# nytdevansh/Optimized-Sparse-Retrieval-for-High-Performance-RAG-Pipelines

Hardware: AMD Instinct MI355X
Metric: queries/sec + achieved HBM GB/s, batch BM25 top-k=100 (higher is better)
Workload: dtype f32

## Files before the change

include/sparse_rx.h:

```cpp
#ifndef SPARSE_RX_H
#define SPARSE_RX_H

#include <stdint.h>

#ifdef __cplusplus
extern "C" {
#endif

#define SRX_VERSION 301

typedef enum {
    SRX_OK = 0,
    SRX_ERR_INVALID = -1,
    SRX_ERR_HIP = -2,
    SRX_ERR_NOMEM = -3,
    SRX_ERR_NODEVICE = -4
} srx_status;

typedef enum {
    SRX_VAL_F32 = 0,
    SRX_VAL_F16 = 1
} srx_val_type;

#define SRX_MAX_K 1024
#define SRX_MAX_TILE_LOG2 14
#define SRX_BLOCK_PAD 256

typedef struct {
    int32_t device;
    int32_t val_type;
    int64_t n_docs;
    int64_t vocab;
    int64_t nnz;
    int64_t n_blocks;
    int64_t doc_base;
    int32_t tile_log2;
    int32_t n_tiles;
    int32_t unit_tiles;
    int32_t reserved0;
    const int64_t *term_ptr;
    const int32_t *post;
    const int32_t *tile_skip;
    const float *idf;
    const float *term_bound;
    const int32_t *post16;
} srx_index_desc;

typedef struct srx_index srx_index;

typedef enum {
    SRX_DBG_TIER2_ONLY = 8,
    SRX_DBG_NO_TERM_BOUND = 16,
    SRX_DBG_NO_FLAT_TILES = 128,
    SRX_DBG_BLOCK_MERGE = 256,
    SRX_DBG_NO_WAVE_DENSE = 2048,
    SRX_DBG_WAVE_DENSE_MASKED = 4096,
    SRX_DBG_WAVE_DENSE_GENERAL = 8192,
    SRX_DBG_ALL = SRX_DBG_TIER2_ONLY | SRX_DBG_NO_TERM_BOUND | SRX_DBG_NO_FLAT_TILES | SRX_DBG_BLOCK_MERGE | SRX_DBG_NO_WAVE_DENSE |
                  SRX_DBG_WAVE_DENSE_MASKED | SRX_DBG_WAVE_DENSE_GENERAL
} srx_debug_bits;

typedef struct {
    int32_t supertile_log2;
    int32_t target_blocks;
    int32_t profile;
    int32_t reserved;
    int32_t unit_tiles;
} srx_search_opts;

int srx_version(void);
const char *srx_last_error(void);
int srx_limits(int32_t *h_out4);
int srx_device_count(void);

int srx_index_create(const srx_index_desc *h_desc, srx_index **h_out);
void srx_index_destroy(srx_index *ix);
int srx_index_set_opts(srx_index *ix, const srx_search_opts *h_opts);

int64_t srx_search_workspace_bytes(const srx_index *ix, int32_t nq, int32_t k);

int srx_search(srx_index *ix, const int32_t *q_ptr, const int32_t *q_term, const float *q_weight, int32_t nq,
               int32_t k, int32_t *out_doc, float *out_score, int32_t *out_count, void *workspace,
               int64_t workspace_bytes, void *stream);

int64_t srx_merge_workspace_bytes(int32_t nq, int32_t n_lists, int32_t k);
int srx_merge_topk(int32_t device, const int32_t *in_doc, const float *in_score, const int32_t *in_count,
                   int32_t nq, int32_t n_lists, int32_t k, int32_t gathered, int32_t *out_doc, float *out_score,
                   int32_t *out_count, void *workspace, int64_t workspace_bytes, void *stream);

int srx_merge_topk_packed(int32_t device, const int32_t *packed, int32_t nq, int32_t n_lists, int32_t k,
                          int32_t *out_doc, float *out_score, int32_t *out_count, void *workspace,
                          int64_t workspace_bytes, void *stream);

int srx_search_packed(srx_index *ix, const int32_t *q_ptr, const int32_t *q_term, const float *q_weight, int32_t nq,
                      int32_t k, int32_t *out_packed, void *workspace, int64_t workspace_bytes, void *stream);
int srx_merge_topk_packed_out(int32_t device, const int32_t *packed, int32_t nq, int32_t n_lists, int32_t k,
                              int32_t *out_packed, void *workspace, int64_t workspace_bytes, void *stream);

int srx_search_after(srx_index *ix, const int32_t *q_ptr, const int32_t *q_term, const float *q_weight, int32_t nq,
                     int32_t k, const int32_t *after_doc, const float *after_score, int32_t *out_doc, float *out_score,
                     int32_t *out_count, void *workspace, int64_t workspace_bytes, void *stream);
int srx_search_after_packed(srx_index *ix, const int32_t *q_ptr, const int32_t *q_term, const float *q_weight, int32_t nq,
                            int32_t k, const int32_t *after_doc, const float *after_score, int32_t *out_packed,
                            void *workspace, int64_t workspace_bytes, void *stream);


int srx_build_impacts(int32_t device, const float *tf, const int32_t *post_doc, const float *doc_len, int64_t nnz,
                      double k1, double b, double avgdl, float *out_impact, void *stream);

int srx_build_tile_skip(int32_t device, const int64_t *term_ptr, const int32_t *post_doc, int64_t vocab,
                        int32_t n_tiles, int32_t tile_log2, int32_t *out_skip, void *stream);

int32_t srx_auto_unit_tiles(int64_t n_docs, int64_t vocab, int64_t nnz, int32_t tile_log2);

int srx_build_blocks(int32_t device, int32_t val_type, const int64_t *term_ptr, const int32_t *post_term,
                     const int32_t *post_doc, const void *post_val, const int32_t *skip, const int64_t *runpad,
                     int64_t vocab, int64_t nnz, int32_t n_tiles, int32_t tile_log2, int32_t unit_tiles, int32_t *out_post,
                     int32_t *out_skip, int64_t *out_term_ptr, int64_t n_blocks, void *stream);

int srx_build_sum_duplicates(int32_t device, const int64_t *first, int64_t n_groups, const float *val, float *out_sum, void *stream);

int srx_build_term_bounds(int32_t device, int32_t val_type, const int64_t *term_ptr, const void *post_val, int64_t vocab,
                          const int32_t *ks, int32_t nk, float *out_bound, int32_t *neg_flag, void *stream);

int srx_build_compact(int32_t device, int32_t val_type, const int32_t *post, int64_t n_blocks_total, int32_t tile_log2,
                      int32_t unit_tiles, int32_t *out_post16, void *stream);

int srx_memcpy_async(void *dst, const void *src, int64_t bytes, void *stream);

int64_t srx_dense_workspace_bytes(int32_t nq, int64_t n_docs, int32_t k);
int srx_dense_search_i8(int32_t device, const int8_t *corpus, const float *corpus_scale, int64_t n_docs, int32_t dim,
                        const int8_t *queries, const float *query_scale, int32_t nq, int32_t k, int64_t doc_base,
                        int32_t *out_doc, float *out_score, int32_t *out_count, void *workspace, int64_t workspace_bytes,
                        void *stream);
int64_t srx_dense_packed_bytes(int64_t n_rows, int32_t dim);
int srx_dense_pack_i8(int32_t device, const int8_t *rows, int64_t n_rows, int32_t dim, void *out_packed, void *stream);
int srx_dense_search_i8_packed(int32_t device, const void *corpus_packed, const float *corpus_scale, int64_t n_docs, int32_t dim,
                               const int8_t *queries, const float *query_scale, int32_t nq, int32_t k, int64_t doc_base,
                               int32_t *out_doc, float *out_score, int32_t *out_count, void *workspace,
                               int64_t workspace_bytes, void *stream);

int64_t srx_dense_f32_workspace_bytes(int32_t nq, int64_t n_docs, int32_t k);
int srx_dense_search_f32(int32_t device, const float *emb, int64_t n_docs, int32_t dim, const float *queries, int32_t nq,
                         int32_t k, int64_t doc_base, int32_t *out_doc, float *out_score, int32_t *out_count,
                         void *workspace, int64_t workspace_bytes, void *stream, float score_offset);

int srx_dense_search_u8(int32_t device, const uint8_t *corpus, const float *corpus_scales, int64_t n_docs, int32_t dim,
                        const float *queries, int32_t nq, int32_t k, int64_t doc_base, int32_t *out_doc, float *out_score,
                        int32_t *out_count, void *workspace, int64_t workspace_bytes, void *stream);

typedef enum {
    SRX_FUSE_WEIGHTED = 0,
    SRX_FUSE_RRF = 1
} srx_fuse_mode;
int srx_fuse_topk(int32_t device, const int32_t *a_doc, const float *a_score, const int32_t *a_count, int32_t ka,
                  const int32_t *b_doc, const float *b_score, const int32_t *b_count, int32_t kb, int32_t nq, int32_t k,
                  int32_t mode, float weight_a, float weight_b, float rrf_c, int32_t *out_doc, float *out_score,
                  int32_t *out_count, void *stream);

int srx_score_docs(const srx_index_desc *h_desc, const int32_t *q_ptr, const int32_t *q_term, const float *q_weight, int32_t nq,
                   const int32_t *cand_doc, const int32_t *cand_count, int32_t m, float *out_score, void *stream);

int srx_profile_read(srx_index *ix, float *h_ms4);

#ifdef __cplusplus
}
#endif
#endif
```

optimized-sparse-retrieval-for-high-performance-rag-pipelines_amd/_capi.py:

```python
from __future__ import annotations

import ctypes
import os
import shutil
import subprocess
from typing import Optional

_PKG_DIR = os.path.dirname(os.path.abspath(__file__))
_ROOT = os.path.dirname(_PKG_DIR)
LIB_PATH = os.path.join(_PKG_DIR, "libsparse_rx.so")
CSRC_DIR = os.path.join(_PKG_DIR, "csrc")
SOURCES = ["wave_kernel.hip", "tier2_kernel.hip", "merge.hip", "build.hip", "sparse_rx.hip", "dense.hip", "fuse.hip",
           "score_docs.hip"]
SRC_PATH = os.path.join(CSRC_DIR, "wave_kernel.hip")
INCLUDE_DIR = os.path.join(_ROOT, "include")

HIPCC_FLAGS = ["--offload-arch=gfx950", "-O3", "-ffp-contract=off", "-fPIC", "-fvisibility=hidden", "-std=c++17"]

SRX_VAL_F32, SRX_VAL_F16 = 0, 1
SRX_FUSE_WEIGHTED, SRX_FUSE_RRF = 0, 1
SRX_MAX_K = 1024


class SparseRxUnavailable(RuntimeError):
    """libsparse_rx.so is not built / not loadable (the HIP engine is mandatory)."""


class SparseRxError(RuntimeError):
    """A C-ABI call returned a negative status."""


class IndexDesc(ctypes.Structure):
    _fields_ = [("device", ctypes.c_int32), ("val_type", ctypes.c_int32), ("n_docs", ctypes.c_int64),
                ("vocab", ctypes.c_int64), ("nnz", ctypes.c_int64), ("n_blocks", ctypes.c_int64), ("doc_base", ctypes.c_int64),
                ("tile_log2", ctypes.c_int32), ("n_tiles", ctypes.c_int32), ("unit_tiles", ctypes.c_int32),
                ("reserved0", ctypes.c_int32), ("term_ptr", ctypes.c_void_p), ("post", ctypes.c_void_p),
                ("tile_skip", ctypes.c_void_p), ("idf", ctypes.c_void_p), ("term_bound", ctypes.c_void_p),
                ("post16", ctypes.c_void_p)]


class SearchOpts(ctypes.Structure):
    _fields_ = [("supertile_log2", ctypes.c_int32), ("target_blocks", ctypes.c_int32), ("profile", ctypes.c_int32),
                ("reserved", ctypes.c_int32), ("unit_tiles", ctypes.c_int32)]


_VP, _I32, _I64, _DBL = ctypes.c_void_p, ctypes.c_int32, ctypes.c_int64, ctypes.c_double
SYMBOLS = {
    "srx_version": (ctypes.c_int, []),
    "srx_last_error": (ctypes.c_char_p, []),
    "srx_limits": (ctypes.c_int, [ctypes.POINTER(_I32)]),
    "srx_device_count": (ctypes.c_int, []),
    "srx_index_create": (ctypes.c_int, [ctypes.POINTER(IndexDesc), ctypes.POINTER(_VP)]),
    "srx_index_destroy": (None, [_VP]),
    "srx_index_set_opts": (ctypes.c_int, [_VP, ctypes.POINTER(SearchOpts)]),
    "srx_search_workspace_bytes": (_I64, [_VP, _I32, _I32]),
    "srx_search": (ctypes.c_int, [_VP, _VP, _VP, _VP, _I32, _I32, _VP, _VP, _VP, _VP, _I64, _VP]),
    "srx_search_after": (ctypes.c_int, [_VP, _VP, _VP, _VP, _I32, _I32, _VP, _VP, _VP, _VP, _VP, _VP, _I64, _VP]),
    "srx_search_after_packed": (ctypes.c_int, [_VP, _VP, _VP, _VP, _I32, _I32, _VP, _VP, _VP, _VP, _I64, _VP]),
    "srx_merge_workspace_bytes": (_I64, [_I32, _I32, _I32]),
    "srx_merge_topk": (ctypes.c_int, [_I32, _VP, _VP, _VP, _I32, _I32, _I32, _I32, _VP, _VP, _VP, _VP, _I64, _VP]),
    "srx_merge_topk_packed": (ctypes.c_int, [_I32, _VP, _I32, _I32, _I32, _VP, _VP, _VP, _VP, _I64, _VP]),
    "srx_search_packed": (ctypes.c_int, [_VP, _VP, _VP, _VP, _I32, _I32, _VP, _VP, _I64, _VP]),
    "srx_merge_topk_packed_out": (ctypes.c_int, [_I32, _VP, _I32, _I32, _I32, _VP, _VP, _I64, _VP]),
    "srx_dense_workspace_bytes": (_I64, [_I32, _I64, _I32]),
    "srx_dense_search_i8": (ctypes.c_int, [_I32, _VP, _VP, _I64, _I32, _VP, _VP, _I32, _I32, _I64, _VP, _VP, _VP, _VP, _I64, _VP]),
    "srx_dense_packed_bytes": (_I64, [_I64, _I32]),
    "srx_dense_pack_i8": (ctypes.c_int, [_I32, _VP, _I64, _I32, _VP, _VP]),
    "srx_dense_search_i8_packed": (ctypes.c_int, [_I32, _VP, _VP, _I64, _I32, _VP, _VP, _I32, _I32, _I64, _VP, _VP, _VP, _VP, _I64, _VP]),
    "srx_dense_f32_workspace_bytes": (_I64, [_I32, _I64, _I32]),
    "srx_dense_search_f32": (ctypes.c_int, [_I32, _VP, _I64, _I32, _VP, _I32, _I32, _I64, _VP, _VP, _VP, _VP, _I64, _VP, ctypes.c_float]),
    "srx_dense_search_u8": (ctypes.c_int, [_I32, _VP, _VP, _I64, _I32, _VP, _I32, _I32, _I64, _VP, _VP, _VP, _VP, _I64, _VP]),
    "srx_fuse_topk": (ctypes.c_int, [_I32, _VP, _VP, _VP, _I32, _VP, _VP, _VP, _I32, _I32, _I32, _I32, ctypes.c_float, ctypes.c_float,
                                     ctypes.c_float, _VP, _VP, _VP, _VP]),
    "srx_score_docs": (ctypes.c_int, [ctypes.POINTER(IndexDesc), _VP, _VP, _VP, _I32, _VP, _VP, _I32, _VP, _VP]),
    "srx_build_impacts": (ctypes.c_int, [_I32, _VP, _VP, _VP, _I64, _DBL, _DBL, _DBL, _VP, _VP]),
    "srx_build_tile_skip": (ctypes.c_int, [_I32, _VP, _VP, _I64, _I32, _I32, _VP, _VP]),
    "srx_memcpy_async": (ctypes.c_int, [_VP, _VP, _I64, _VP]),
    "srx_auto_unit_tiles": (_I32, [_I64, _I64, _I64, _I32]),
    "srx_build_blocks": (ctypes.c_int, [_I32, _I32, _VP, _VP, _VP, _VP, _VP, _VP, _I64, _I64, _I32, _I32, _I32, _VP, _VP, _VP, _I64, _VP]),
    "srx_build_compact": (ctypes.c_int, [_I32, _I32, _VP, _I64, _I32, _I32, _VP, _VP]),
    "srx_build_term_bounds": (ctypes.c_int, [_I32, _I32, _VP, _VP, _I64, _VP, _I32, _VP, _VP, _VP]),
    "srx_build_sum_duplicates": (ctypes.c_int, [_I32, _VP, _I64, _VP, _VP, _VP]),
    "srx_profile_read": (ctypes.c_int, [_VP, ctypes.POINTER(ctypes.c_float)]),
}

_lib: Optional[ctypes.CDLL] = None


def kernel_sources_sha256() -> str:
    import hashlib
    h = hashlib.sha256()
    for f in ["wave_kernel.hip", "tier2_kernel.hip", "merge.hip", "srx_common.h"]:
        with open(os.path.join(CSRC_DIR, f), "rb") as fh:
            h.update(fh.read())
    return h.hexdigest()


def _deps():
    return [os.path.join(CSRC_DIR, f) for f in SOURCES] + [os.path.join(CSRC_DIR, "srx_common.h"),
                                                            os.path.join(INCLUDE_DIR, "sparse_rx.h")]


def build_library(force: bool = False, verbose: bool = False) -> str:
    if not force and os.path.exists(LIB_PATH) and os.path.getmtime(LIB_PATH) >= max(os.path.getmtime(p) for p in _deps()):
        return LIB_PATH
    hipcc = shutil.which("hipcc") or "/opt/rocm/bin/hipcc"
    if not os.path.exists(hipcc):
        raise SparseRxUnavailable("hipcc not found: cannot build libsparse_rx.so")
    objdir = os.path.join(CSRC_DIR, "build")
    os.makedirs(objdir, exist_ok=True)
    newest_hdr = max(os.path.getmtime(os.path.join(CSRC_DIR, "srx_common.h")), os.path.getmtime(os.path.join(INCLUDE_DIR, "sparse_rx.h")))
    procs, objs = [], []
    for f in SOURCES:
        src, obj = os.path.join(CSRC_DIR, f), os.path.join(objdir, f.replace(".hip", ".o"))
        objs.append(obj)
        if not force and os.path.exists(obj) and os.path.getmtime(obj) >= max(os.path.getmtime(src), newest_hdr):
            continue
        cmd = [hipcc, *HIPCC_FLAGS, f"-I{INCLUDE_DIR}", f"-I{CSRC_DIR}", "-c", "-o", obj, src]
        if verbose:
            print(" ".join(cmd))
        procs.append((f, subprocess.Popen(cmd)))
    for f, p in procs:
        if p.wait() != 0:
            raise subprocess.CalledProcessError(p.returncode, f"hipcc -c {f}")
    cmd = [hipcc, "--offload-arch=gfx950", "-shared", "-fPIC", "-fvisibility=hidden", "-o", LIB_PATH, *objs]
    if verbose:
        print(" ".join(cmd))
    subprocess.run(cmd, check=True)
    return LIB_PATH


def lib() -> ctypes.CDLL:
    global _lib
    if _lib is not None:
        return _lib
    if not os.path.exists(LIB_PATH):
        raise SparseRxUnavailable(
            f"{LIB_PATH} is missing: build it with `python -c 'import __graft_entry__ as g; g.build()'` "
            "(hipcc --offload-arch=gfx950).  There is no CPU fallback.")
    try:
        L = ctypes.CDLL(LIB_PATH)
    except OSError as e:
        raise SparseRxUnavailable(f"cannot load {LIB_PATH}: {e}") from e
    for name, (res, args) in SYMBOLS.items():
        try:
            f = getattr(L, name)
        except AttributeError as e:
            raise SparseRxUnavailable(f"{LIB_PATH} does not export {name}") from e
        f.restype = res
        f.argtypes = args
    _lib = L
    return L


def check(rc: int, what: str) -> int:
    if rc < 0:
        msg = lib().srx_last_error()
        text = msg.decode("utf-8", "replace") if msg else ""
        if rc == -1:
            raise ValueError(f"{what}: {text}")
        raise SparseRxError(f"{what} failed ({rc}): {text}")
    return rc


def limits():
    out = (ctypes.c_int32 * 4)()
    check(lib().srx_limits(out), "srx_limits")
    return {"max_k": out[0], "max_tile_log2": out[1], "hash_cap": out[2], "threads": out[3]}
```

optimized-sparse-retrieval-for-high-performance-rag-pipelines_amd/csrc/sparse_rx.hip:

```cpp

#include "srx_common.h"

thread_local char srx_g_err[512] = "";

#define SRX_TRY(expr)                  \
    do {                               \
        const int rc_ = (expr);        \
        if (rc_ != SRX_OK) return rc_; \
    } while (0)

namespace {
constexpr int PROF_SLOTS = 256;
constexpr int PROF_EVENTS = 4;
struct SearchProfile {
    hipEvent_t *ev;
    hipEvent_t *cur;
    int n;
    int64_t calls;
    int64_t searches;

    int begin(int every) {
        cur = nullptr;
        if (every <= 0 || (searches++ % every) != 0) return SRX_OK;
        if (!ev) {
            ev = new (std::nothrow) hipEvent_t[PROF_EVENTS * PROF_SLOTS];
            if (!ev) return fail(SRX_ERR_NOMEM, "srx_search: host allocation failed%s");
            for (int i = 0; i < PROF_EVENTS * PROF_SLOTS; ++i) HIP_TRY(hipEventCreate(&ev[i]));
        }
        cur = ev + PROF_EVENTS * (int)(calls % PROF_SLOTS);
        return SRX_OK;
    }
    int mark(int i, hipStream_t stream) {
        if (cur) HIP_TRY(hipEventRecord(cur[i], stream));
        return SRX_OK;
    }
    void end() {
        if (!cur) return;
        ++calls;
        if (n < PROF_SLOTS) ++n;
    }
    int read(float *h_ms4) {
        if (n == 0 || !ev) return fail(SRX_ERR_INVALID, "srx_profile_read: no profiled srx_search has run%s");
        static constexpr int FROM[4] = {0, 1, 2, 0}, TO[4] = {1, 2, 3, 3};
        double acc[4] = {0, 0, 0, 0};
        for (int i = 0; i < n; ++i) {
            const hipEvent_t *e = ev + PROF_EVENTS * (int)((calls - 1 - i) % PROF_SLOTS);
            HIP_TRY(hipEventSynchronize(e[3]));
            for (int j = 0; j < 4; ++j) {
                float ms = 0;
                HIP_TRY(hipEventElapsedTime(&ms, e[FROM[j]], e[TO[j]]));
                acc[j] += ms;
            }
        }
        for (int j = 0; j < 4; ++j) h_ms4[j] = (float)(acc[j] / n);
        const int averaged = n;
        n = 0;
        return averaged;
    }
    void destroy() {
        if (!ev) return;
        for (int i = 0; i < PROF_EVENTS * PROF_SLOTS; ++i) (void)hipEventDestroy(ev[i]);
        delete[] ev;
    }
};
}

struct srx_index {
    srx_index_desc d;
    srx_search_opts opts;
    SearchProfile prof;
    int *h_hint;
    int *d_hint;
};

SRX_API int srx_version(void) { return SRX_VERSION; }
SRX_API const char *srx_last_error(void) { return g_err; }

SRX_API int srx_limits(int32_t *h_out4) {
    if (!h_out4) return fail(SRX_ERR_INVALID, "srx_limits: null output%s");
    h_out4[0] = KMAX;
    h_out4[1] = SRX_MAX_TILE_LOG2;
    h_out4[2] = HASH_CAP;
    h_out4[3] = THREADS;
    return SRX_OK;
}

SRX_API int srx_device_count(void) {
    int n = 0;
    hipError_t e = hipGetDeviceCount(&n);
    if (e != hipSuccess) return fail(SRX_ERR_NODEVICE, "hipGetDeviceCount: %s", hipGetErrorString(e));
    return n;
}

SRX_API int srx_index_create(const srx_index_desc *d, srx_index **out) {
    if (!d || !out) return fail(SRX_ERR_INVALID, "srx_index_create: null argument%s");
    if (d->n_docs <= 0 || d->n_docs >= 0x7FFFFFFFll) return fail(SRX_ERR_INVALID, "srx_index_create: n_docs out of range%s");
    if (d->doc_base < 0 || d->doc_base + d->n_docs >= 0x7FFFFFFFll)
        return fail(SRX_ERR_INVALID, "srx_index_create: doc_base + n_docs must fit int32%s");
    if (d->vocab <= 0 || d->nnz < 0) return fail(SRX_ERR_INVALID, "srx_index_create: bad vocab / nnz%s");
    if (d->tile_log2 < 6 || d->tile_log2 > SRX_MAX_TILE_LOG2)
        return fail(SRX_ERR_INVALID, "srx_index_create: tile_log2 must be in [6, 14]%s");
    const int64_t nt = (d->n_docs + (1ll << d->tile_log2) - 1) >> d->tile_log2;
    if (d->n_tiles != nt) return fail(SRX_ERR_INVALID, "srx_index_create: n_tiles != ceil(n_docs / 2^tile_log2)%s");
    if (d->val_type != SRX_VAL_F32 && d->val_type != SRX_VAL_F16) return fail(SRX_ERR_INVALID, "srx_index_create: bad val_type%s");
    if (d->unit_tiles < 1 || d->unit_tiles > MAX_TPS) return fail(SRX_ERR_INVALID, "srx_index_create: unit_tiles must be in [1, 64]%s");
    if (d->n_blocks < 0 || d->n_blocks * 4 < d->nnz) return fail(SRX_ERR_INVALID, "srx_index_create: n_blocks does not cover nnz%s");
    if (!d->term_ptr || !d->tile_skip || !d->idf || (!d->post && !d->post16))
        return fail(SRX_ERR_INVALID, "srx_index_create: null index array%s");
    if (!d->post && ((int64_t)d->unit_tiles << d->tile_log2) > W_UNIT_MAX_DOCS)
        return fail(SRX_ERR_INVALID, "srx_index_create: an index without canonical blocks needs units of <= 49152 docs (the compact copy)%s");
    int ndev = 0;
    HIP_TRY(hipGetDeviceCount(&ndev));
    if (d->device < 0 || d->device >= ndev) return fail(SRX_ERR_NODEVICE, "srx_index_create: device ordinal not visible%s");
    srx_index *ix = new (std::nothrow) srx_index();
    if (!ix) return fail(SRX_ERR_NOMEM, "srx_index_create: host allocation failed%s");
    ix->d = *d;
    int *h = nullptr, *dev = nullptr;
    const bool pinned = hipSetDevice(d->device) == hipSuccess && hipHostMalloc((void **)&h, 64, hipHostMallocMapped) == hipSuccess;
    if (pinned && hipHostGetDevicePointer((void **)&dev, h, 0) == hipSuccess) {
        h[0] = -1;
        ix->h_hint = h;
        ix->d_hint = dev;
    } else {
        if (pinned) (void)hipHostFree(h);
        (void)hipGetLastError();
    }
    *out = ix;
    return SRX_OK;
}

SRX_API void srx_index_destroy(srx_index *ix) {
    if (!ix) return;
    ix->prof.destroy();
    if (ix->h_hint) (void)hipHostFree(ix->h_hint);
    delete ix;
}

SRX_API int srx_index_set_opts(srx_index *ix, const srx_search_opts *o) {
    if (!ix || !o) return fail(SRX_ERR_INVALID, "srx_index_set_opts: null argument%s");
    if (o->supertile_log2 != 0 && (o->supertile_log2 < ix->d.tile_log2 || o->supertile_log2 > ix->d.tile_log2 + 6))
        return fail(SRX_ERR_INVALID, "srx_index_set_opts: supertile_log2 must be in [tile_log2, tile_log2+6]%s");
    if (o->unit_tiles < 0 || o->unit_tiles > MAX_TPS) return fail(SRX_ERR_INVALID, "srx_index_set_opts: unit_tiles must be in [0, 64]%s");
    if (o->target_blocks < 0) return fail(SRX_ERR_INVALID, "srx_index_set_opts: target_blocks < 0%s");
    if (o->reserved & ~SRX_DBG_ALL)
        return fail(SRX_ERR_INVALID, "srx_index_set_opts: reserved takes only the bits 8, 16, 128, 256, 2048, 4096, 8192%s");
    ix->opts = *o;
    return SRX_OK;
}

namespace {
struct Plan {
    int tpu, n_super, n_splits, n_whole, ovf_words, lists_per_q;
};

Plan make_plan(const srx_index *ix, int nq, int k) {
    Plan p;
    const srx_index_desc &d = ix->d;
    int tpu;
    if (ix->opts.unit_tiles > 0) {
        tpu = ix->opts.unit_tiles;
    } else if (ix->opts.supertile_log2 != 0) {
        tpu = 1 << (ix->opts.supertile_log2 - d.tile_log2);
    } else {
        tpu = d.unit_tiles;
    }
    if (tpu < 1) tpu = 1;
    if (tpu > MAX_TPS) tpu = MAX_TPS;
    p.tpu = tpu;
    p.n_super = (int)((d.n_tiles + tpu - 1) / tpu);
    const int target = ix->opts.target_blocks > 0 ? ix->opts.target_blocks : 3072;
    int ns = target / (nq > 0 ? nq : 1);
    int n_whole = 0;
    if (nq > target) {
        n_whole = nq / target * target;
        const int tail = nq - n_whole;
        ns = tail > 0 ? target / tail : 1;
        if (ns > 4) ns = 4;
        if (ns < 2) ns = 2;
        if (tail == 0) ns = 1;
    }
    if (ns < 1) ns = 1;
    if (ns > p.n_super) ns = p.n_super;
    const int cap = (MERGE_NPT * THREADS) / (2 * (k > 0 ? k : 1));
    if (ns > cap) ns = cap;
    if (ns < 1) ns = 1;
    if (ns == 1) n_whole = 0;
    p.n_splits = ns;
    p.n_whole = n_whole;
    p.ovf_words = (p.n_super + 31) / 32;
    p.lists_per_q = 2 * ns;
    return p;
}
}

namespace {
struct SearchWs {
    int32_t *cand_doc;
    float *cand_score;
    int32_t *cand_count;
    unsigned *ovf;
    unsigned *done;
    int *work;
    int64_t lists, items;
    int64_t bytes;
};
SearchWs search_ws(void *base, const Plan &p, int nq, int k) {
    SearchWs w;
    w.lists = (int64_t)nq * p.lists_per_q;
    w.items = (int64_t)p.n_whole + (int64_t)(nq - p.n_whole) * p.n_splits;
    w.cand_doc = (int32_t *)base;
    w.cand_score = (float *)(w.cand_doc + w.lists * k);
    w.cand_count = (int32_t *)(w.cand_score + w.lists * k);
    w.ovf = (unsigned *)(w.cand_count + w.lists);
    w.done = w.ovf + w.items * p.ovf_words;
    w.work = (int *)(w.done + (nq - p.n_whole));
    w.bytes = (int64_t)((char *)(w.work + 1 + w.items) - (char *)base) + 256;
    return w;
}
}

SRX_API int64_t srx_search_workspace_bytes(const srx_index *ix, int32_t nq, int32_t k) {
    if (!ix || nq < 0 || k <= 0 || k > KMAX) return fail(SRX_ERR_INVALID, "srx_search_workspace_bytes: bad argument%s");
    return search_ws(nullptr, make_plan(ix, nq, k), nq, k).bytes;
}

namespace {
IndexView index_view(const srx_index *ix, bool after) {
    const srx_index_desc &d = ix->d;
    IndexView v;
    v.term_ptr = d.term_ptr; v.post = d.post; v.post16 = d.post16; v.tile_skip = d.tile_skip; v.idf = d.idf;
    v.term_bound = ((ix->opts.reserved & SRX_DBG_NO_TERM_BOUND) || after) ? nullptr : d.term_bound;
    v.n_docs = d.n_docs; v.vocab = d.vocab; v.zero_block = d.n_blocks;
    v.tile_log2 = d.tile_log2; v.n_tiles = d.n_tiles; v.unit_tiles = d.unit_tiles;
    return v;
}

int search_impl(srx_index *ix, const int32_t *q_ptr, const int32_t *q_term, const float *q_weight, int32_t nq,
                int32_t k, const srx_rows &out, void *workspace, int64_t workspace_bytes, void *stream_v,
                const int32_t *after_doc = nullptr, const float *after_score = nullptr) {
    if (!ix) return fail(SRX_ERR_INVALID, "srx_search: null index%s");
    if ((after_doc == nullptr) != (after_score == nullptr)) return fail(SRX_ERR_INVALID, "srx_search_after: after_doc and after_score go together%s");
    if (nq < 0 || k <= 0 || k > KMAX) return fail(SRX_ERR_INVALID, "srx_search: need nq >= 0 and 1 <= k <= 1024%s");
    if (nq == 0) return SRX_OK;
    if (!q_ptr || !out.doc || !out.score || !out.count) return fail(SRX_ERR_INVALID, "srx_search: null query / output pointer%s");
    const Plan p = make_plan(ix, nq, k);
    const SearchWs w = search_ws(workspace, p, nq, k);
    if (!workspace || workspace_bytes < w.bytes) return fail(SRX_ERR_NOMEM, "srx_search: workspace too small%s");
    hipStream_t stream = (hipStream_t)stream_v;
    HIP_TRY(hipSetDevice(ix->d.device));
    if (ix->d.post == nullptr && p.tpu != ix->d.unit_tiles)
        return fail(SRX_ERR_INVALID, "srx_search: this index keeps no canonical blocks: a unit other than the one it was built for cannot be served%s");
    if (w.lists > 0x7FFFFFFFll) return fail(SRX_ERR_INVALID, "srx_search: nq * splits overflows the grid%s");

    const bool tier2_only = (ix->opts.reserved & SRX_DBG_TIER2_ONLY) != 0 || after_score != nullptr || p.tpu != ix->d.unit_tiles;
    srx_score_launch sl;
    srx_wave_launch &a = sl.w;
    a.ix = index_view(ix, after_score != nullptr);
    a.q_ptr = q_ptr; a.q_term = q_term; a.q_weight = q_weight;
    a.nq = nq; a.k = k; a.n_splits = p.n_splits; a.n_whole = p.n_whole; a.n_super = p.n_super;
    a.dbg = ix->opts.reserved | (tier2_only ? SRX_DBG_TIER2_ONLY : 0);
    a.ovf = w.ovf; a.ovf_words = p.ovf_words; a.lists_per_q = p.lists_per_q; a.work = w.work; a.done = w.done;
    a.cand_doc = w.cand_doc; a.cand_score = w.cand_score; a.cand_count = w.cand_count;
    a.doc_base = ix->d.doc_base; a.out_doc = out.doc; a.out_score = out.score; a.out_count = out.count;
    a.out_row_stride = out.row_stride; a.out_cnt_stride = out.cnt_stride;
    sl.tpu = p.tpu; sl.after_doc = after_doc; sl.after_score = after_score; sl.hint = ix->d_hint;

    SRX_TRY(ix->prof.begin(ix->opts.profile));
    HIP_TRY(hipMemsetAsync(w.done, 0, (size_t)(1 + (nq - p.n_whole)) * 4, stream));
    SRX_TRY(ix->prof.mark(0, stream));
    SRX_TRY(srx_launch_wave_kernel(sl.w, ix->d.val_type, w.items, stream));
    SRX_TRY(ix->prof.mark(1, stream));
    const int hint = ix->h_hint ? *(volatile int *)ix->h_hint : -1;
    const int64_t t2_full = w.items < 1024 ? w.items : 1024;
    const bool t2_small = hint == 0 && t2_full > 128 && !tier1_serves_nothing(a.ix, k, p.tpu, a.dbg);
    SRX_TRY(srx_launch_score_kernel(sl, ix->d.val_type, (unsigned)(t2_small ? 128 : t2_full), stream));
    SRX_TRY(ix->prof.mark(2, stream));
    if (nq > p.n_whole)
        SRX_TRY(srx_launch_final_merge(srx_plain_rows(w.cand_doc, w.cand_score, w.cand_count, k), nq, p.lists_per_q, k, 0, ix->d.doc_base,
                                       out, nullptr, p.n_whole, 1, (a.dbg & SRX_DBG_BLOCK_MERGE) != 0, stream));
    SRX_TRY(ix->prof.mark(3, stream));
    ix->prof.end();
    return SRX_OK;
}
}

SRX_API int srx_search(srx_index *ix, const int32_t *q_ptr, const int32_t *q_term, const float *q_weight, int32_t nq,
                       int32_t k, int32_t *out_doc, float *out_score, int32_t *out_count, void *workspace,
                       int64_t workspace_bytes, void *stream_v) {
    return search_impl(ix, q_ptr, q_term, q_weight, nq, k, srx_plain_rows(out_doc, out_score, out_count, k), workspace,
                       workspace_bytes, stream_v);
}

SRX_API int srx_search_packed(srx_index *ix, const int32_t *q_ptr, const int32_t *q_term, const float *q_weight,
                              int32_t nq, int32_t k, int32_t *out_packed, void *workspace, int64_t workspace_bytes,
                              void *stream_v) {
    if (!out_packed || k <= 0) return fail(SRX_ERR_INVALID, "srx_search_packed: bad argument%s");
    return search_impl(ix, q_ptr, q_term, q_weight, nq, k, srx_packed_rows<float>(out_packed, k), workspace, workspace_bytes, stream_v);
}

SRX_API int srx_search_after(srx_index *ix, const int32_t *q_ptr, const int32_t *q_term, const float *q_weight, int32_t nq,
                             int32_t k, const int32_t *after_doc, const float *after_score, int32_t *out_doc, float *out_score,
                             int32_t *out_count, void *workspace, int64_t workspace_bytes, void *stream_v) {
    if (!after_doc || !after_score) return fail(SRX_ERR_INVALID, "srx_search_after: null bound arrays%s");
    return search_impl(ix, q_ptr, q_term, q_weight, nq, k, srx_plain_rows(out_doc, out_score, out_count, k), workspace,
                       workspace_bytes, stream_v, after_doc, after_score);
}

SRX_API int srx_search_after_packed(srx_index *ix, const int32_t *q_ptr, const int32_t *q_term, const float *q_weight,
                                    int32_t nq, int32_t k, const int32_t *after_doc, const float *after_score,
                                    int32_t *out_packed, void *workspace, int64_t workspace_bytes, void *stream_v) {
    if (!out_packed || k <= 0 || !after_doc || !after_score) return fail(SRX_ERR_INVALID, "srx_search_after_packed: bad argument%s");
    return search_impl(ix, q_ptr, q_term, q_weight, nq, k, srx_packed_rows<float>(out_packed, k), workspace, workspace_bytes, stream_v,
                       after_doc, after_score);
}

SRX_API int srx_profile_read(srx_index *ix, float *h_ms4) {
    if (!ix || !h_ms4) return fail(SRX_ERR_INVALID, "srx_profile_read: null argument%s");
    return ix->prof.read(h_ms4);
}

SRX_API int srx_memcpy_async(void *dst, const void *src, int64_t bytes, void *stream_v) {
    if (bytes < 0 || (bytes > 0 && (!dst || !src))) return fail(SRX_ERR_INVALID, "srx_memcpy_async: bad argument%s");
    if (bytes == 0) return SRX_OK;
    HIP_TRY(hipMemcpyAsync(dst, src, (size_t)bytes, hipMemcpyDefault, (hipStream_t)stream_v));
    return SRX_OK;
}
```

Before: 9.319 million.

## Add new tier-1 wave kernel with prefetch pipeline and bitmap duplicate detection

Adds a separate tier-1 scoring kernel, launched by default in place of the previous wave kernel, which stays reachable through a new debug bit. The new kernel reads query-term metadata with a scalar prologue and prefetches tile-skip bounds and posting blocks two supertiles ahead. Duplicate docs are found with an LDS bitmap plus atomicOr, and dense units are sent to tier 2. The aim is to hide load latency and lower per-unit overhead, at the price of a large new code path with its own register and LDS pressure.

```diff
diff --git a/include/sparse_rx.h b/include/sparse_rx.h
--- a/include/sparse_rx.h
+++ b/include/sparse_rx.h
@@ -56,8 +56,9 @@
     SRX_DBG_NO_WAVE_DENSE = 2048,
     SRX_DBG_WAVE_DENSE_MASKED = 4096,
     SRX_DBG_WAVE_DENSE_GENERAL = 8192,
+    SRX_DBG_TIER1_PREVIOUS = 16384,
     SRX_DBG_ALL = SRX_DBG_TIER2_ONLY | SRX_DBG_NO_TERM_BOUND | SRX_DBG_NO_FLAT_TILES | SRX_DBG_BLOCK_MERGE | SRX_DBG_NO_WAVE_DENSE |
-                  SRX_DBG_WAVE_DENSE_MASKED | SRX_DBG_WAVE_DENSE_GENERAL
+                  SRX_DBG_WAVE_DENSE_MASKED | SRX_DBG_WAVE_DENSE_GENERAL | SRX_DBG_TIER1_PREVIOUS
 } srx_debug_bits;
 
 typedef struct {
diff --git a/optimized-sparse-retrieval-for-high-performance-rag-pipelines_amd/_capi.py b/optimized-sparse-retrieval-for-high-performance-rag-pipelines_amd/_capi.py
--- a/optimized-sparse-retrieval-for-high-performance-rag-pipelines_amd/_capi.py
+++ b/optimized-sparse-retrieval-for-high-performance-rag-pipelines_amd/_capi.py
@@ -10,7 +10,7 @@
 _ROOT = os.path.dirname(_PKG_DIR)
 LIB_PATH = os.path.join(_PKG_DIR, "libsparse_rx.so")
 CSRC_DIR = os.path.join(_PKG_DIR, "csrc")
-SOURCES = ["wave_kernel.hip", "tier2_kernel.hip", "merge.hip", "build.hip", "sparse_rx.hip", "dense.hip", "fuse.hip",
+SOURCES = ["tier1_kernel.hip", "wave_kernel.hip", "tier2_kernel.hip", "merge.hip", "build.hip", "sparse_rx.hip", "dense.hip", "fuse.hip",
            "score_docs.hip"]
 SRC_PATH = os.path.join(CSRC_DIR, "wave_kernel.hip")
 INCLUDE_DIR = os.path.join(_ROOT, "include")
diff --git a/optimized-sparse-retrieval-for-high-performance-rag-pipelines_amd/csrc/sparse_rx.hip b/optimized-sparse-retrieval-for-high-performance-rag-pipelines_amd/csrc/sparse_rx.hip
--- a/optimized-sparse-retrieval-for-high-performance-rag-pipelines_amd/csrc/sparse_rx.hip
+++ b/optimized-sparse-retrieval-for-high-performance-rag-pipelines_amd/csrc/sparse_rx.hip
@@ -1,5 +1,7 @@
 
 #include "srx_common.h"
+
+int srx_launch_tier1_kernel(const srx_wave_launch &a, int val_type, int64_t blocks, hipStream_t stream);
 
 thread_local char srx_g_err[512] = "";
 
@@ -143,7 +145,7 @@
     if (o->unit_tiles < 0 || o->unit_tiles > MAX_TPS) return fail(SRX_ERR_INVALID, "srx_index_set_opts: unit_tiles must be in [0, 64]%s");
     if (o->target_blocks < 0) return fail(SRX_ERR_INVALID, "srx_index_set_opts: target_blocks < 0%s");
     if (o->reserved & ~SRX_DBG_ALL)
-        return fail(SRX_ERR_INVALID, "srx_index_set_opts: reserved takes only the bits 8, 16, 128, 256, 2048, 4096, 8192%s");
+        return fail(SRX_ERR_INVALID, "srx_index_set_opts: reserved takes only the bits 8, 16, 128, 256, 2048, 4096, 8192, 16384%s");
     ix->opts = *o;
     return SRX_OK;
 }
@@ -268,7 +270,10 @@
     SRX_TRY(ix->prof.begin(ix->opts.profile));
     HIP_TRY(hipMemsetAsync(w.done, 0, (size_t)(1 + (nq - p.n_whole)) * 4, stream));
     SRX_TRY(ix->prof.mark(0, stream));
-    SRX_TRY(srx_launch_wave_kernel(sl.w, ix->d.val_type, w.items, stream));
+    if (a.dbg & SRX_DBG_TIER1_PREVIOUS)
+        SRX_TRY(srx_launch_wave_kernel(sl.w, ix->d.val_type, w.items, stream));
+    else
+        SRX_TRY(srx_launch_tier1_kernel(sl.w, ix->d.val_type, w.items, stream));
     SRX_TRY(ix->prof.mark(1, stream));
     const int hint = ix->h_hint ? *(volatile int *)ix->h_hint : -1;
     const int64_t t2_full = w.items < 1024 ? w.items : 1024;
diff --git a/optimized-sparse-retrieval-for-high-performance-rag-pipelines_amd/csrc/tier1_kernel.hip b/optimized-sparse-retrieval-for-high-performance-rag-pipelines_amd/csrc/tier1_kernel.hip
--- /dev/null
+++ b/optimized-sparse-retrieval-for-high-performance-rag-pipelines_amd/csrc/tier1_kernel.hip
@@ -0,0 +1,478 @@
+
+#include "srx_common.h"
+
+namespace {
+
+enum { U_OK = 0, U_DENSE = 1, U_FULL = 2 };
+
+constexpr int W_DEPTH = 2;
+struct WaveShared2 {
+    static constexpr int LCAP = W1_LCAP;
+    static constexpr bool HIST_ALIASES_ZEROED_LDS = true;
+    union {
+        unsigned bm[W_BM_WORDS];
+        unsigned hist[256];
+    };
+    unsigned lbits[LCAP];
+    int ldoc[LCAP];
+};
+static_assert(sizeof(WaveShared2) * 4 * W_WAVES_PER_EU <= 160 * 1024, "tier-1 LDS per wave does not allow the waves per SIMD the kernel is built for");
+
+constexpr int W_RP = W_R / 2;
+static_assert(W_R == 12, "score() dispatches units of 1, 2 or 3 load steps");
+__device__ __forceinline__ unsigned slot_id(const unsigned (&dp)[W_RP], int r) {
+    return (r & 1) ? dp[r >> 1] >> 16 : dp[r >> 1] & 0xFFFFu;
+}
+template <int NR>
+__device__ __forceinline__ int lane_reg(const unsigned (&dp)[W_RP], int rs, int src) {
+    unsigned w;
+    switch (rs >> 1) {
+#define SRX_CASE(i) \
+    case i:         \
+        w = (unsigned)__builtin_amdgcn_readlane((int)dp[(i) < NR / 2 ? (i) : 0], src); \
+        break;
+        SRX_CASE(1) SRX_CASE(2) SRX_CASE(3) SRX_CASE(4) SRX_CASE(5) SRX_CASE(6) SRX_CASE(7)
+#undef SRX_CASE
+        default:
+            w = (unsigned)__builtin_amdgcn_readlane((int)dp[0], src);
+    }
+    return (int)((rs & 1) ? w >> 16 : w & 0xFFFFu);
+}
+
+template <typename VT>
+__global__ __launch_bounds__(64) __attribute__((amdgpu_waves_per_eu(W_WAVES_PER_EU))) void srx_tier1_kernel(const srx_wave_launch a) {
+    __shared__ WaveShared2 S;
+    constexpr int BW = CompactWords<VT>::value;
+    const IndexView &ix = a.ix;
+    const int lane = threadIdx.x;
+    const int k = a.k;
+    int q, split, nsq;
+    decode_item((int)blockIdx.x, a.n_whole, a.n_splits, q, split, nsq);
+    if (q >= a.nq) return;
+    const int64_t list = (int64_t)q * a.lists_per_q + split;
+    const int t0 = a.q_ptr[q];
+    const int nt = a.q_ptr[q + 1] - t0;
+    const int n_terms_all = a.q_ptr[a.nq];
+    const int tpu = ix.unit_tiles;
+    unsigned *const my_ovf = a.ovf + (int64_t)blockIdx.x * a.ovf_words;
+    for (int w = lane; w < a.ovf_words; w += 64) __hip_atomic_store(&my_ovf[w], 0u, __ATOMIC_RELAXED, __HIP_MEMORY_SCOPE_AGENT);
+    if (lane == 0) a.cand_count[(int64_t)q * a.lists_per_q + a.n_splits + split] = 0;
+    if (nt == 0 || tier1_cannot_serve(ix, nt, k, tpu, a.dbg)) {
+        if (lane == 0) {
+            a.cand_count[list] = 0;
+            if (nt > 0) a.work[1 + atomicAdd(&a.work[0], 1)] = (int)blockIdx.x;
+        }
+        if (nt == 0 && nsq == 1 && a.out_doc != nullptr) {
+            for (int i = lane; i < k; i += 64) {
+                a.out_doc[(int64_t)q * a.out_row_stride + i] = -1;
+                a.out_score[(int64_t)q * a.out_row_stride + i] = 0.0f;
+            }
+            if (lane == 0) {
+                a.out_count[(int64_t)q * a.out_cnt_stride] = 0;
+                a.cand_count[list] = -1;
+            }
+        }
+        return;
+    }
+    const int su_lo = (int)(((int64_t)a.n_super * split) / nsq);
+    const int su_hi = (int)(((int64_t)a.n_super * (split + 1)) / nsq);
+    const int row = ix.n_tiles + 1;
+
+    for (int i = lane; i < W_BM_WORDS / 4; i += 64) reinterpret_cast<uint4 *>(S.bm)[i] = make_uint4(0u, 0u, 0u, 0u);
+    wsync();
+    WaveTopk tk = {0u, 0u};
+    bool flagged = false;
+    int lg = 0;
+    while ((1 << lg) < nt) ++lg;
+
+    auto run = [&](auto lconst) __attribute__((always_inline)) {
+        constexpr int LPT_LOG2 = decltype(lconst)::value;
+        constexpr int LPT = 1 << LPT_LOG2;
+        const int tslot = lane >> LPT_LOG2;
+        const int jl = lane & (LPT - 1);
+        const bool has_term = tslot < nt;
+        int64_t tblk = 0;
+        unsigned skip_boff = 0;
+        float my_idf = 0.f, my_qw = 0.f, my_bnd = 0.f;
+        constexpr int NBQ = W_DEPTH + 2;
+        int bq[NBQ];
+        const int col = bound_column(k);
+        const bool use_bound = ix.term_bound != nullptr && col >= 0;
+        constexpr bool SCALAR_PROLOGUE = LPT_LOG2 >= 3;
+        if constexpr (SCALAR_PROLOGUE) {
+            constexpr int NTS = 64 >> LPT_LOG2;
+            int s_term[NTS];
+            float s_qwt[NTS];
+            typedef int srx_ivec __attribute__((ext_vector_type(NTS < 2 ? 2 : NTS), aligned(4)));
+            typedef float srx_fvec __attribute__((ext_vector_type(NTS < 2 ? 2 : NTS), aligned(4)));
+            if (t0 + (NTS < 2 ? 2 : NTS) <= n_terms_all) {
+                const srx_ivec tv = *(const SRX_CONSTANT srx_ivec *)(a.q_term + t0);
+                const srx_fvec wv = *(const SRX_CONSTANT srx_fvec *)(a.q_weight + t0);
+#pragma unroll
+                for (int i = 0; i < NTS; ++i) {
+                    s_term[i] = tv[i];
+                    s_qwt[i] = wv[i];
+                }
+            } else {
+#pragma unroll
+                for (int i = 0; i < NTS; ++i) {
+                    s_term[i] = cload_i32(a.q_term + t0 + min(i, nt - 1));
+                    s_qwt[i] = cload_f32(a.q_weight + t0 + min(i, nt - 1));
+                }
+            }
+            auto pick = [](unsigned m, unsigned x, unsigned old) __attribute__((always_inline)) { return (x & m) | (old & ~m); };
+            unsigned v_tlo = 0, v_thi = 0, v_idf = 0, v_qw = 0, v_bnd = 0, v_bq[2] = {0u, 0u};
+            constexpr int TB = NTS < 4 ? NTS : 4;
+            auto batches = [&](auto with_bound) __attribute__((always_inline)) {
+                constexpr bool WB = decltype(with_bound)::value != 0;
+#pragma unroll
+                for (int h = 0; h < NTS; h += TB) {
+                    int64_t s_tp[TB];
+                    float s_idf[TB], s_b[TB];
+                    int s_q0[TB], s_q1[TB];
+#pragma unroll
+                    for (int j = 0; j < TB; ++j) {
+                        const int ti = s_term[h + j];
+                        s_tp[j] = cload_i64(ix.term_ptr + ti);
+                        s_idf[j] = cload_f32(ix.idf + ti);
+                        s_b[j] = WB ? cload_f32(ix.term_bound + (int64_t)ti * 4 + col) : 0.0f;
+                        s_q0[j] = cload_i32(ix.tile_skip + (int64_t)ti * row + min(su_lo * tpu, ix.n_tiles));
+                        s_q1[j] = cload_i32(ix.tile_skip + (int64_t)ti * row + min((su_lo + 1) * tpu, ix.n_tiles));
+                    }
+                    __builtin_amdgcn_sched_barrier(0);
+#pragma unroll
+                    for (int j = 0; j < TB; ++j) {
+                        const int ti = s_term[h + j];
+                        const unsigned m = tslot == h + j ? 0xFFFFFFFFu : 0u;
+                        const int64_t tb = s_tp[j] >> 2;
+                        v_tlo = pick(m, (unsigned)(tb & 0xFFFFFFFFll), v_tlo);
+                        v_thi = pick(m, (unsigned)(tb >> 32), v_thi);
+                        skip_boff = pick(m, ((unsigned)ti * (unsigned)row) << 2, skip_boff);
+                        v_idf = pick(m, __float_as_uint(s_idf[j]), v_idf);
+                        v_qw = pick(m, __float_as_uint(s_qwt[h + j]), v_qw);
+                        v_bnd = pick(m, __float_as_uint(s_b[j]), v_bnd);
+                        v_bq[0] = pick(m, (unsigned)s_q0[j], v_bq[0]);
+                        v_bq[1] = pick(m, (unsigned)s_q1[j], v_bq[1]);
+                    }
+                    __builtin_amdgcn_sched_barrier(0);
+                }
+            };
+            if (use_bound)
+                batches(IntC<1>{});
+            else
+                batches(IntC<0>{});
+            bq[0] = (int)v_bq[0];
+            bq[1] = (int)v_bq[1];
+            tblk = (int64_t)(((unsigned long long)v_thi << 32) | v_tlo);
+            my_idf = __uint_as_float(v_idf);
+            my_qw = __uint_as_float(v_qw);
+            my_bnd = __uint_as_float(v_bnd);
+        } else if (has_term) {
+            const int term = a.q_term[t0 + tslot];
+            tblk = ix.term_ptr[term] >> 2;
+            skip_boff = ((unsigned)term * (unsigned)row) << 2;
+            my_idf = ix.idf[term];
+            my_qw = a.q_weight[t0 + tslot];
+            if (use_bound) my_bnd = ix.term_bound[(int64_t)term * 4 + col];
+        }
+        {
+            float bnd = 0.0f;
+            if (use_bound && has_term && my_idf > 0.0f && my_qw > 0.0f) bnd = 0.0f + (my_bnd * my_idf) * my_qw;
+            const bool neg = has_term && (my_idf < 0.0f || my_qw < 0.0f);
+            const unsigned t0bits = wave_max(__float_as_uint(bnd > 0.0f ? bnd : 0.0f));
+            tk.tau = (__ballot(neg) != 0ull) ? 0u : uniu(t0bits);
+        }
+        unsigned tau_seen = 0xFFFFFFFFu;
+        float vthr = 0.0f;
+        const int32_t *const zblk = ix.post16 + (ix.zero_block + lane) * BW;
+        const int32_t *const tpost = ix.post16 + (tblk + jl) * BW;
+
+        auto bound = [&](int j) __attribute__((always_inline)) -> int {
+            return gload_i32(reinterpret_cast<const int32_t *>(reinterpret_cast<const char *>(ix.tile_skip) +
+                                                               (size_t)(skip_boff + ((unsigned)min(j * tpu, ix.n_tiles) << 2))));
+        };
+
+        auto issue = [&](int lo, int len, unsigned (&d)[W_RP], float (&v)[W_R]) __attribute__((always_inline)) {
+            const int32_t *p = tpost + (int64_t)lo * BW;
+            const int rem = len - jl;
+#pragma unroll
+            for (int s4 = 0; s4 < W_R / 4; ++s4) {
+                const int off = (s4 << LPT_LOG2) * BW;
+                const bool ok = (s4 << LPT_LOG2) < rem;
+                unsigned dd[2];
+                float vv[4];
+                load_block16p((ok ? p : zblk) + off, VT(), dd, vv);
+                d[2 * s4] = dd[0];
+                d[2 * s4 + 1] = dd[1];
+#pragma unroll
+                for (int c = 0; c < 4; ++c) v[4 * s4 + c] = vv[c];
+            }
+        };
+
+        auto process = [&](auto nrc, int ubase, unsigned (&d)[W_RP], float (&v)[W_R]) __attribute__((always_inline)) -> int {
+            constexpr int NR = decltype(nrc)::value;
+            const unsigned count0 = tk.count = uniu(tk.count);
+            if (count0 + (unsigned)W_DUPCAP + 1u > (unsigned)WaveShared2::LCAP) return U_FULL;
+            unsigned adr[NR], t[NR];
+#pragma unroll
+            for (int r = 0; r < NR; ++r) {
+                const unsigned w = d[r >> 1];
+                adr[r] = (w >> ((r & 1) ? 19 : 3)) & W_BM_ADR_MASK;
+                unsigned one;
+                asm("v_min_u32 %0, 1, %1" : "=v"(one) : "v"(__float_as_uint(v[r])));
+                const unsigned bit = one << (((r & 1) ? w >> 16 : w) & 31u);
+                t[r] = atomicOr(reinterpret_cast<unsigned *>(reinterpret_cast<char *>(S.bm) + adr[r]), bit) & bit;
+            }
+            unsigned acc = 0;
+#pragma unroll
+            for (int r = 0; r < NR; ++r) acc |= t[r];
+            bool dense = false;
+            const bool anydup = __ballot(acc != 0u) != 0ull;
+#pragma unroll
+            for (int r = 0; r < NR; ++r) *reinterpret_cast<unsigned *>(reinterpret_cast<char *>(S.bm) + adr[r]) = 0u;
+            if (anydup) {
+                unsigned fm = 0;
+#pragma unroll
+                for (int r = 0; r < NR; ++r) {
+                    unsigned one;
+                    asm("v_min_u32 %0, 1, %1" : "=v"(one) : "v"(t[r]));
+                    fm |= one << r;
+                }
+                unsigned n_res = 0;
+                unsigned long long m = __ballot(fm != 0u);
+                while (m != 0ull) {
+                    const int src = __ffsll((long long)m) - 1;
+                    const unsigned fms = (unsigned)__builtin_amdgcn_readlane((int)fm, src);
+                    const int rs = __ffs((int)fms) - 1;
+                    const int dd = lane_reg<NR>(d, rs, src);
+                    float myv = 0.0f;
+#pragma unroll
+                    for (int r2 = 0; r2 < NR; ++r2) {
+                        const bool hit = (int)slot_id(d, r2) == dd;
+                        myv = hit ? v[r2] : myv;
+                        v[r2] = hit ? 0.0f : v[r2];
+                    }
+                    const float myc = 0.0f + (myv * my_idf) * my_qw;
+                    unsigned long long mm = __ballot(myv != 0.0f);
+                    float sum = 0.0f;
+                    while (mm != 0ull) {
+                        const int l2 = __ffsll((long long)mm) - 1;
+                        sum = sum + __uint_as_float((unsigned)__builtin_amdgcn_readlane((int)__float_as_uint(myc), l2));
+                        mm &= mm - 1ull;
+                    }
+                    const unsigned b = uniu(__float_as_uint(sum));
+                    if (b - 1u < 0x7F800000u && b >= tk.tau) {
+                        if (lane == 0) {
+                            S.lbits[tk.count] = b;
+                            S.ldoc[tk.count] = ubase + dd;
+                        }
+                        tk.count = uniu(tk.count + 1u);
+                    }
+                    if (++n_res > (unsigned)W_DUPCAP) {
+                        dense = true;
+                        tk.count = count0;
+                        break;
+                    }
+                    fm = (lane == src) ? (fm & (fm - 1u)) : fm;
+                    m = __ballot(fm != 0u);
+                }
+            }
+            if (dense) return U_DENSE;
+            if (tk.tau != tau_seen) {
+                tau_seen = tk.tau;
+                const float tau_f = __uint_as_float(max(tau_seen, 1u));
+                vthr = (my_idf > 0.0f && my_qw > 0.0f) ? fmaxf(((tau_f / my_qw) / my_idf) * 0.99999f, __uint_as_float(1u))
+                                                     : __builtin_inff();
+            }
+            float vmax = v[0];
+#pragma unroll
+            for (int r = 1; r + 1 < NR; r += 2) vmax = fmaxf(fmaxf(vmax, v[r]), v[r + 1]);
+            if constexpr (NR % 2 == 0) vmax = fmaxf(vmax, v[NR - 1]);
+            const bool anycand = __ballot(vmax >= vthr) != 0ull;
+            if (anycand) {
+#pragma unroll
+                for (int r = 0; r < NR; ++r) {
+                    const bool pass = v[r] >= vthr;
+                    if (__ballot(pass) != 0ull) {
+                        const float c = 0.0f + (v[r] * my_idf) * my_qw;
+                        const unsigned b = __float_as_uint(c);
+                        const bool cand = pass & (c > 0.0f) & (b >= tk.tau);
+                        const unsigned long long m2 = __ballot(cand);
+                        const unsigned n2 = (unsigned)__popcll(m2);
+                        if (tk.count + n2 > (unsigned)WaveShared2::LCAP) {
+                            tk.count = count0;
+                            return U_FULL;
+                        }
+                        if (cand) {
+                            const unsigned pz = tk.count + lane_rank(m2);
+                            S.lbits[pz] = b;
+                            S.ldoc[pz] = ubase + (int)slot_id(d, r);
+                        }
+                        tk.count = uniu(tk.count + n2);
+                    }
+                }
+            }
+            return U_OK;
+        };
+
+        auto flag_tier2 = [&](int su) __attribute__((always_inline)) {
+            if (lane == 0) atomicOr(&my_ovf[su >> 5], 1u << (su & 31));
+        };
+
+        auto score = [&](int su, int steps, unsigned (&d)[W_RP], float (&v)[W_R]) __attribute__((always_inline)) -> bool {
+            flagged |= steps > W_R / 4;
+            if (steps > W_R / 4) {
+                flag_tier2(su);
+            } else if (steps > 0) {
+                int rc;
+                const int ubase = (su * tpu) << ix.tile_log2;
+                if (steps == 3)
+                    rc = process(IntC<12>{}, ubase, d, v);
+                else if (steps == 2)
+                    rc = process(IntC<8>{}, ubase, d, v);
+                else
+                    rc = process(IntC<4>{}, ubase, d, v);
+                flagged |= rc == U_DENSE;
+                if (rc == U_DENSE) flag_tier2(su);
+                return rc == U_FULL;
+            }
+            return false;
+        };
+        int su_issue = su_lo;
+        auto fetch = [&](unsigned (&d)[W_RP], float (&v)[W_R]) __attribute__((always_inline)) -> int {
+            const int len = (has_term && su_issue < su_hi) ? (bq[1] - bq[0]) >> 2 : 0;
+            int steps = 0;
+#pragma unroll
+            for (int s4 = 0; s4 <= W_R / 4; ++s4) {
+                const unsigned long long any = __ballot(len > (s4 << LPT_LOG2));
+                steps += (int)min((unsigned)any | (unsigned)(any >> 32), 1u);
+            }
+            issue(bq[0] >> 2, steps > W_R / 4 ? 0 : len, d, v);
+#pragma unroll
+            for (int i = 0; i < NBQ - 1; ++i) bq[i] = bq[i + 1];
+            ++su_issue;
+            bq[NBQ - 1] = bound(su_issue + NBQ - 1);
+            return steps;
+        };
+        constexpr int DEPTH = W_DEPTH;
+        int su_start = su_lo;
+        for (;;) {
+            su_start = uni(su_start);
+            tk.count = uniu(tk.count), tk.tau = uniu(tk.tau);
+            su_issue = su_start;
+            const bool first_start = SCALAR_PROLOGUE && su_start == su_lo;
+#pragma unroll
+            for (int i = 0; i < NBQ; ++i) {
+                const int bi = bound(su_start + i);
+                bq[i] = (i < 2 && first_start) ? bq[i] : bi;
+            }
+            unsigned dS[DEPTH][W_RP];
+            float vS[DEPTH][W_R];
+            int st[DEPTH];
+#pragma unroll
+            for (int j = 0; j < DEPTH - 1; ++j) st[j] = fetch(dS[j], vS[j]);
+            st[DEPTH - 1] = 0;
+            int su_full = -1;
+            for (int su = su_start; su < su_hi && su_full < 0; su += DEPTH) {
+#pragma unroll
+                for (int j = 0; j < DEPTH; ++j) {
+                    if ((j == 0 || su + j < su_hi) && su_full < 0) {
+                        st[(j + DEPTH - 1) % DEPTH] = fetch(dS[(j + DEPTH - 1) % DEPTH], vS[(j + DEPTH - 1) % DEPTH]);
+                        if (score(su + j, st[j], dS[j], vS[j])) su_full = su + j;
+                    }
+                }
+            }
+            su_full = uni(su_full);
+            tk.count = uniu(tk.count);
+            if (su_full < 0) break;
+            if (tk.count > (unsigned)k) {
+                tk.tau = uniu(wave_list_select(S, tk.count, k));
+                tk.count = (unsigned)k;
+                su_start = su_full;
+            } else {
+                flagged = true;
+                flag_tier2(su_full);
+                su_start = su_full + 1;
+            }
+        }
+    };
+    switch (6 - lg) {
+        case 0: run(IntC<0>{}); break;
+        case 1: run(IntC<1>{}); break;
+        case 2: run(IntC<2>{}); break;
+        case 3: run(IntC<3>{}); break;
+        case 4: run(IntC<4>{}); break;
+        case 5: run(IntC<5>{}); break;
+        default: run(IntC<6>{}); break;
+    }
+    unsigned count = tk.count;
+    if (count > (unsigned)k) {
+        wave_list_select(S, count, k);
+        count = (unsigned)k;
+    }
+    if (nsq == 1 && !flagged && a.out_doc != nullptr) {
+        wave_rank_emit(S, reinterpret_cast<unsigned long long *>(S.bm), count, k, a.doc_base, a.out_doc + (int64_t)q * a.out_row_stride,
+                       a.out_score + (int64_t)q * a.out_row_stride);
+        if (lane == 0) {
+            a.out_count[(int64_t)q * a.out_cnt_stride] = (int)count;
+            a.cand_count[list] = -1;
+        }
+        return;
+    }
+    const int64_t o = list * k;
+    for (unsigned i = lane; i < count; i += 64) {
+        __hip_atomic_store(&a.cand_doc[o + i], S.ldoc[i], __ATOMIC_RELAXED, __HIP_MEMORY_SCOPE_AGENT);
+        __hip_atomic_store(reinterpret_cast<unsigned *>(&a.cand_score[o + i]), S.lbits[i], __ATOMIC_RELAXED, __HIP_MEMORY_SCOPE_AGENT);
+    }
+    if (lane == 0) {
+        __hip_atomic_store(&a.cand_count[list], (int)count, __ATOMIC_RELAXED, __HIP_MEMORY_SCOPE_AGENT);
+        if (flagged) a.work[1 + atomicAdd(&a.work[0], 1)] = (int)blockIdx.x;
+    }
+    if (nsq > 1 && a.done != nullptr && a.out_doc != nullptr) {
+        asm volatile("s_waitcnt vmcnt(0)" ::: "memory");
+        __builtin_amdgcn_fence(__ATOMIC_RELEASE, "workgroup");
+        unsigned old = 0;
+        if (lane == 0) old = atomicAdd(&a.done[q - a.n_whole], 1u + (flagged ? 0x10000u : 0u));
+        old = uniu(old);
+        if ((old & 0xFFFFu) + 1u == (unsigned)nsq && (old >> 16) == 0u && !flagged) {
+            const int64_t l0 = (int64_t)q * a.lists_per_q;
+            for (int s2 = 0; s2 < nsq; ++s2) {
+                if (s2 == split) continue;
+                const unsigned c2 = (unsigned)min(max(__hip_atomic_load(&a.cand_count[l0 + s2], __ATOMIC_RELAXED, __HIP_MEMORY_SCOPE_AGENT), 0), k);
+                if (count + c2 > (unsigned)WaveShared2::LCAP) {
+                    wave_list_select(S, count, k);
+                    count = (unsigned)k;
+                }
+                for (unsigned i = lane; i < c2; i += 64) {
+                    S.ldoc[count + i] = __hip_atomic_load(&a.cand_doc[(l0 + s2) * k + i], __ATOMIC_RELAXED, __HIP_MEMORY_SCOPE_AGENT);
+                    S.lbits[count + i] = __hip_atomic_load(reinterpret_cast<const unsigned *>(&a.cand_score[(l0 + s2) * k + i]), __ATOMIC_RELAXED,
+                                                           __HIP_MEMORY_SCOPE_AGENT);
+                }
+                count += c2;
+                wsync();
+            }
+            if (count > (unsigned)k) {
+                wave_list_select(S, count, k);
+                count = (unsigned)k;
+            }
+            wave_rank_emit(S, reinterpret_cast<unsigned long long *>(S.bm), count, k, a.doc_base, a.out_doc + (int64_t)q * a.out_row_stride,
+                           a.out_score + (int64_t)q * a.out_row_stride);
+            if (lane == 0) {
+                a.out_count[(int64_t)q * a.out_cnt_stride] = (int)count;
+                a.cand_count[l0] = -1;
+            }
+        }
+    }
+}
+
+}
+
+int srx_launch_tier1_kernel(const srx_wave_launch &a, int val_type, int64_t blocks, hipStream_t stream) {
+    if (blocks <= 0) return SRX_OK;
+    if (val_type == SRX_VAL_F32)
+        hipLaunchKernelGGL((srx_tier1_kernel<float>), dim3((unsigned)blocks), dim3(64), 0, stream, a);
+    else
+        hipLaunchKernelGGL((srx_tier1_kernel<__half>), dim3((unsigned)blocks), dim3(64), 0, stream, a);
+    HIP_TRY(hipGetLastError());
+    return SRX_OK;
+}
```

After: 9.301 million, median of 3. No clear change (-0.2%).
